# wexiangis/wmix

Hardware: AMD Instinct MI355X
Metric: 10 ms frames/s (higher is better)
Workload: dtype f32

## Files before the change

include/wmix_amd.h:

```cpp
#ifndef WMIX_AMD_H
#define WMIX_AMD_H

#include <stddef.h>
#include <stdint.h>

#ifdef __cplusplus
extern "C" {
#endif

#define WMX_EINVAL (-10001)
#define WMX_ENODEV (-10002)
#define WMX_ESTATE (-10003)
#define WMX_EHIP_BASE (-11000)
#define WMX_IS_HIP_ERROR(rc) ((rc) <= WMX_EHIP_BASE && (rc) > WMX_EHIP_BASE - 10000)

const char *wmx_last_error(void);
int wmx_device_count(void);
int wmx_handle_device(const void *handle);
int wmx_version(void);
const char *wmx_build_info(void);



#define WMX_LAW_A 0
// ... 125 lines not shown
wmx_ns *wmx_chain_ns(wmx_chain *h);
wmx_aec *wmx_chain_aec(wmx_chain *h);
wmx_agc *wmx_chain_agc(wmx_chain *h);
wmx_vad *wmx_chain_vad(wmx_chain *h);

typedef struct wmx_aecm wmx_aecm;
int wmx_aecm_create(wmx_aecm **out, int n_streams, int chn, int freq, int interval_ms);
int wmx_aecm_destroy(wmx_aecm *h);
int wmx_aecm_packet_samples(const wmx_aecm *h);
int wmx_aecm_state_bytes(const wmx_aecm *h);
int wmx_aecm_run(wmx_aecm *h, int mode, const int16_t *d_far, long far_packet_stride, const int16_t *d_near,
                 int16_t *d_out, int n_packets, long stream_stride, long packet_stride, int delay_ms, void *stream);
int wmx_aecm_create_cohorts(wmx_aecm **out, int n_streams, int chn, int freq, int interval_ms, int n_cohorts);
int wmx_aecm_cohorts(const wmx_aecm *h);
int wmx_aecm_reset_cohort(wmx_aecm *h, int cohort, void *stream);
int wmx_aecm_add_cohort(wmx_aecm *h, int *cohort, void *stream);
int wmx_aecm_retire_cohort(wmx_aecm *h, int cohort);
int wmx_aecm_coalesce(wmx_aecm *h, int max_pairs, int32_t *merged_from, int32_t *merged_into, int cap, int *n_merged, void *stream);
int wmx_aecm_live_cohorts(const wmx_aecm *h);
int wmx_aec_cohort_key(const wmx_aec *h, int cohort, int32_t *key11);
int wmx_aecm_cohort_key(const wmx_aecm *h, int cohort, int32_t *key8);
int wmx_aecm_reset_streams(wmx_aecm *h, const int32_t *idx, int n, int cohort, void *stream);
int wmx_aecm_set_active(wmx_aecm *h, const uint8_t *host_mask, void *stream);
int wmx_aecm_stream_state_bytes(const wmx_aecm *h);
int wmx_aecm_export_stream(wmx_aecm *h, int stream_index, void *host_blob);
int wmx_aecm_import_stream(wmx_aecm *h, int stream_index, const void *host_blob, int cohort);
int wmx_aecm_cohort_state_bytes(const wmx_aecm *h);
int wmx_aecm_export_cohort(wmx_aecm *h, int cohort, void *host_blob);
int wmx_aecm_import_cohort(wmx_aecm *h, int cohort, const void *host_blob);
int wmx_aecm_run_cohorts(wmx_aecm *h, int mode, const int16_t *d_far, long far_packet_stride, long far_group_stride,
                         const int16_t *d_near, int16_t *d_out, int n_packets, long stream_stride, long packet_stride,
                         const int32_t *delay_ms, const uint8_t *cohort_on, int32_t *cohort_rc, void *stream);
wmx_nsx *wmx_chain_nsx(wmx_chain *h);
wmx_aecm *wmx_chain_aecm(wmx_chain *h);

int wmx_pcm_zoom(int inChn, int inFreq, const int16_t *d_in, uint32_t inLen, int outChn, int outFreq, int16_t *d_out,
                 uint32_t out_capacity, long in_stride, long out_stride, int n_streams, uint32_t *out_len, void *stream);
typedef struct wmx_mix wmx_mix;
int wmx_mix_create(wmx_mix **out, int n_groups, int ring_chn, int ring_freq);
int wmx_mix_destroy(wmx_mix *m);
int wmx_mix_set(wmx_mix *m, uint32_t head_off, uint32_t tick, int reduce_mode);
int wmx_mix_set_play_correct(wmx_mix *m, uint32_t bytes);
int wmx_mix_ring_bytes(const wmx_mix *m);
int wmx_mix_load(wmx_mix *m, const int16_t *d_src, uint32_t srcU8Len, int freq, int channels, int sample, int n_src,
                 long group_stride, long source_stride, int reduce, uint32_t *head, uint32_t *tick, void *stream);
#define WMX_MIX_MAX_PARTIES 32
int wmx_mix_load_minus(wmx_mix *m, int parties, const int16_t *d_src, uint32_t srcU8Len, int freq, int channels, int sample,
                       long conf_stride, long source_stride, const uint8_t *d_mute, int reduce, uint32_t *head, uint32_t *tick,
                       void *stream);
int wmx_mix_set_conferences(wmx_mix *m, int n_conf, const int32_t *host_off, const int32_t *host_members, void *stream);
int wmx_mix_conferences(const wmx_mix *m);
int wmx_mix_load_minus_conf(wmx_mix *m, const int16_t *d_src, uint32_t srcU8Len, int freq, int channels, int sample,
                            long source_stride, const uint8_t *d_mute, int reduce, uint32_t *head, uint32_t *tick, void *stream);
int wmx_mix_select_speakers(wmx_mix *m, int parties, const int16_t *d_src, uint32_t srcU8Len, long conf_stride, long source_stride,
                            const uint8_t *d_mute, int max_speakers, uint32_t floor, int decay_shift, uint8_t *d_mute_out, void *stream);
int wmx_mix_select_speakers_conf(wmx_mix *m, const int16_t *d_src, uint32_t srcU8Len, long source_stride, const uint8_t *d_mute,
                                 int max_speakers, uint32_t floor, int decay_shift, uint8_t *d_mute_out, void *stream);
int wmx_mix_reset_speakers(wmx_mix *m, const int32_t *host_idx, int n, void *stream);
int wmx_mix_export_speakers(const wmx_mix *m, uint32_t *host_env, uint8_t *host_speaking, void *stream);
int wmx_mix_drain(wmx_mix *m, int16_t *d_out, uint32_t bytes, long out_stride, void *stream);
int wmx_mix_export(const wmx_mix *m, int group, int16_t *host_ring, uint32_t *head_off, uint32_t *tick);

#define WMX_MFFT_FFT 0
#define WMX_MFFT_FFTR 1
#define WMX_MFFT_IFFT 2
#define WMX_MFFT_IFFTR 3
int wmx_mfft(int kind, int n_batch, unsigned N, const float *d_in_re, const float *d_in_im, float *d_out_re,
             float *d_out_im, float *d_out_af, float *d_out_pf, void *stream);
int wmx_mfft_stream(int n_streams, const float *d_in, unsigned in_len, float *d_pool, unsigned st_len, float *d_out_af,
                    float *d_out_pf, void *stream);

typedef struct wmx_rtp wmx_rtp;
int wmx_rtp_create(wmx_rtp **out, int n_streams, int law);
int wmx_rtp_destroy(wmx_rtp *h);
int wmx_rtp_egress(wmx_rtp *h, int in_chn, int in_freq, const int16_t *d_pcm, uint32_t in_bytes, long pcm_stride, int out_chn,
                   int out_freq, uint8_t *d_packets, long packet_stride, uint32_t *packet_bytes, void *stream);
int wmx_rtp_ingest(int n_streams, const uint8_t *d_packets, long packet_stride, int16_t *d_pcm, long pcm_stride,
                   uint32_t *d_pcm_bytes, uint16_t *d_seq_raw, void *stream);
int wmx_rtp_export(wmx_rtp *h, int stream_index, uint16_t *seq, uint32_t *timestamp);

typedef struct wmx_pipe wmx_pipe;
int wmx_pipe_create(wmx_pipe **out, int n_streams, int slots, int law, int agc_value, unsigned stages);
int wmx_pipe_create_pcm(wmx_pipe **out, int n_streams, int slots, int chn, int freq, int interval_ms, int agc_value, unsigned stages);
int wmx_pipe_create_pcm_calls(wmx_pipe **out, int n_streams, int slots, int chn, int freq, int interval_ms, int agc_value, unsigned stages);
int wmx_pipe_destroy(wmx_pipe *h);
int wmx_pipe_slots(const wmx_pipe *h);
int wmx_pipe_datagram_bytes(const wmx_pipe *h);
uint8_t *wmx_pipe_in(wmx_pipe *h, int slot);
const uint8_t *wmx_pipe_out(wmx_pipe *h, int slot);
int16_t *wmx_pipe_far(wmx_pipe *h, int slot);
int wmx_pipe_submit(wmx_pipe *h, const int16_t *d_far, int *slot, void *stream);
int wmx_pipe_wait(wmx_pipe *h, int slot);
long wmx_pipe_failed_steps(const wmx_pipe *h);
int wmx_pipe_poll(wmx_pipe *h, int slot);
int wmx_pipe_step_resident(wmx_pipe *h, const uint8_t *d_in, long in_stride, const int16_t *d_far, uint8_t *d_out, long out_stride,
                           void *stream);
wmx_chain *wmx_pipe_chain(wmx_pipe *h);
wmx_rtp *wmx_pipe_senders(wmx_pipe *h);

typedef struct wmx_rt wmx_rt;
int wmx_rt_create_pcm(wmx_rt **out, long n_streams, int sub_batch, int slots, int chn, int freq, int interval_ms, int agc_value, unsigned stages);
int wmx_rt_create_rtp(wmx_rt **out, long n_streams, int sub_batch, int slots, int law, int agc_value, unsigned stages);
int wmx_rt_create_pcm_calls(wmx_rt **out, long n_streams, int sub_batch, int slots, int chn, int freq, int interval_ms, int agc_value, unsigned stages);
int wmx_rt_destroy(wmx_rt *h);
int wmx_rt_set_compute_streams(wmx_rt *h, int n);
int wmx_rt_batches(const wmx_rt *h);
int wmx_rt_batch_streams(const wmx_rt *h, int batch);
wmx_pipe *wmx_rt_pipe(wmx_rt *h, int batch);
int16_t *wmx_rt_far(wmx_rt *h, int slot);
int wmx_rt_submit(wmx_rt *h, const int16_t *d_far, int *slot, void *stream);
#define WMX_DROPPED 1
int wmx_rt_try_submit(wmx_rt *h, const int16_t *d_far, int *slot, void *stream);
long wmx_rt_dropped_ticks(const wmx_rt *h);
int wmx_rt_next_slot(const wmx_rt *h);
int wmx_rt_wait(wmx_rt *h);
int wmx_rt_poll(wmx_rt *h);
int wmx_rt_tick(wmx_rt *h, const int16_t *d_far, int *slot, void *stream);
int wmx_rt_step_resident(wmx_rt *h, uint8_t *d_rows, long stride, const int16_t *d_far, uint8_t *d_out, long out_stride, void *stream);

typedef struct wmx_pkgfifo wmx_pkgfifo;
int wmx_pkgfifo_create(wmx_pkgfifo **out, int n_streams, int n_slots, int pkg_bytes, int interval_ms, int frame_bytes);
int wmx_pkgfifo_destroy(wmx_pkgfifo *h);
int wmx_pkgfifo_add(wmx_pkgfifo *h, const uint8_t *d_pkgs, long stride, void *stream);
int wmx_pkgfifo_get(wmx_pkgfifo *h, uint8_t *d_out, long stride, int delayms, void *stream);

typedef struct wmx_tick wmx_tick;
int wmx_tick_create(wmx_tick **out, int n_groups, int rec_per_group, int chn, int freq, int interval_ms, int aec_delay_ms, int agc_value,
                    unsigned stages);
int wmx_tick_destroy(wmx_tick *h);
int wmx_tick_set_stages(wmx_tick *h, unsigned stages, int agc_value);
int wmx_tick_play_ns(wmx_tick *h, int on);
int wmx_tick_rw_test(wmx_tick *h, int on);
int wmx_tick_bridge(wmx_tick *h, int parties);
int wmx_tick_bridge_mute(wmx_tick *h, const uint8_t *host_mask, void *stream);
int wmx_tick_bridge_conferences(wmx_tick *h, int n_conf, const int32_t *host_off, const int32_t *host_members, void *stream);
int wmx_tick_bridge_speakers(wmx_tick *h, int max_speakers, uint32_t floor, int decay_shift);
int wmx_tick_bridge_speaking(wmx_tick *h, uint8_t *host_speaking, uint32_t *host_env, void *stream);
int wmx_tick_set_play_correct(wmx_tick *h, uint32_t bytes);
int wmx_tick_package_samples(const wmx_tick *h);
int wmx_tick_load(wmx_tick *h, const int16_t *d_src, uint32_t srcU8Len, int freq, int channels, int sample, int n_src, long group_stride,
                  long source_stride, int reduce, uint32_t *head, uint32_t *tick, void *stream);
int wmx_tick_play(wmx_tick *h, int16_t *d_play, long play_stride, void *stream);
const int16_t *wmx_tick_far(const wmx_tick *h);
int wmx_tick_record(wmx_tick *h, int16_t *d_rec, long rec_stride, int16_t *d_rec_1x8000, long out_stride, uint32_t out_capacity,
                    uint32_t *out_len, void *stream);
int wmx_tick_run(wmx_tick *h, int16_t *d_play, long play_stride, int16_t *d_rec, long rec_stride, int16_t *d_rec_1x8000, long out_stride,
                 uint32_t out_capacity, uint32_t *out_len, void *stream);
wmx_mix *wmx_tick_mix(wmx_tick *h);
wmx_chain *wmx_tick_chain(wmx_tick *h);
wmx_pkgfifo *wmx_tick_fifo(wmx_tick *h);

int wmx_debug_fft(int kind, int n_batch, void *d_data, int32_t *d_aux, void *stream);
int wmx_debug_ns_libm(int kind, const float *x, float *y, size_t n);
int wmx_debug_div(const float *d_a, const float *d_b, float *d_q_ordinary, float *d_q_ieee, size_t n, void *stream);
int wmx_debug_div_host(const float *a, const float *b, float *q, size_t n);
int wmx_debug_pow(const float *x, const float *e, float *y, size_t n);
int wmx_debug_pow_device(const float *d_x, const float *d_e, float *d_y, size_t n, void *stream);

#ifdef __cplusplus
}
#endif
#endif
```

tools_dev/ns_prof.py:

```python
import sys, ctypes; sys.path.insert(0,'.')
import numpy as np, torch
from wmix_amd import synth, _lib
from wmix_amd.ns import NsBatch
dev=torch.device('cuda:0'); S=int(sys.argv[1]) if len(sys.argv)>1 else 65536
import os
if os.environ.get('WMX_TOOL_LIB'): _lib.LIB_PATH=os.environ['WMX_TOOL_LIB']
lib=_lib.lib(); f=lib.wmx_debug_ns_prof; f.argtypes=[ctypes.c_void_p,ctypes.c_int]
nb=NsBatch(S,1,16000); nf=int(sys.argv[2]) if len(sys.argv)>2 else 260
x=synth.ns_input(7,64,nf,160)
d=torch.from_numpy(np.ascontiguousarray(x.reshape(64,nf,160).transpose(1,0,2))).to(dev).repeat(1,S//64,1).contiguous()
buf=(ctypes.c_ulonglong*16)()
for k in range(nf):
    if k==nf-8: f(buf,1)
    nb.process_packet_major(d[k:k+1])
f(buf,0); v=np.array(buf[:14],dtype=np.float64)
names=['load+window+energy1','fft fwd','spectrum+log','7 sums','noise est (quantiles)','startup/snr loop','3 sums+flat','lrt loop (log)','ksum+prior+exp loop','noise update+wiener','ifft','td+energy2','synth+hb','output']
for n,x in zip(names,v): print('%-24s %8.1f Mcyc %5.1f%%'%(n,x/1e6,100*x/v.sum()))
```

wmix_amd/csrc/ns.hip:

```cpp
#include <cmath>
#include <vector>
#include "stage_life.h"
#include "fft_ooura.h"
#include "libm_dev.h"
#include "ns_layout.h"

namespace wmx {
namespace {

constexpr int kStartupShort = 50;
constexpr int kStartupLong = 200;
constexpr int kHistBins = 1000;
constexpr int kUpdateWindow = 500;
constexpr int kStartBand = 5;

constexpr int kNsWavesPerBlock = 4;

template <int L>
struct NsConstLds {
    FftTables tab;
    float window[L];
    float logi[NsLayout<L>::MP];
    NsLibmTables lm;
};
template <int L>
struct alignas(16) NsWaveLds {
    static constexpr int MP = NsLayout<L>::MP;
    float fa[L];
    float magn[MP], lmagn[MP], noise[MP], snrp[MP], sprob[MP], pause[MP];
    float r0[MP], r1[MP], r2[MP];
#ifdef WMX_NS_PROF
    unsigned long long prof[16];
#endif
};
#ifdef WMX_NS_PROF
__device__ unsigned long long g_ns_prof[16];
#define NS_PROF(i)                                                         \
    do {                                                                   \
        const long long t_now = clock64();                                 \
        if (lane == 0) W.prof[i] += (unsigned long long)(t_now - prof_t0); \
        prof_t0 = clock64();                                               \
    } while (0)
#else
#define NS_PROF(i)
#endif
static_assert(2 * NsLayout<256>::MP >= 256 && 2 * NsLayout<128>::MP >= 128, "r0..r1 must hold L floats");

__device__ __forceinline__ float sat16f(float v) { return v > 32767.f ? 32767.f : (v < -32768.f ? -32768.f : v); }

__device__ __forceinline__ float sum_range(const float *x, int lo, int hi, int lane) {
    float acc = 0.f;
    int i = lo;
#pragma unroll 1
    for (; i < hi && (i & 3); i++) acc += x[i];
#pragma unroll 4
    for (; i + 8 <= hi; i += 8) {
        const float4 a = *reinterpret_cast<const float4 *>(x + i), b = *reinterpret_cast<const float4 *>(x + i + 4);
        acc += a.x;
        acc += a.y;
        acc += a.z;
        acc += a.w;
        acc += b.x;
        acc += b.y;
        acc += b.z;
        acc += b.w;
    }
#pragma unroll 1
    for (; i < hi; i++) acc += x[i];
    return acc;
}

template <int MP4>
__device__ __forceinline__ float sum_lanes(const float *mine) {
    float acc = 0.f;
#pragma unroll 4
    for (int i = 0; i < MP4; i += 2) {
        const float4 a = *reinterpret_cast<const float4 *>(mine + 4 * i);
        acc += a.x;
        acc += a.y;
        acc += a.z;
        acc += a.w;
        if (i + 1 < MP4) {
            const float4 b = *reinterpret_cast<const float4 *>(mine + 4 * i + 4);
            acc += b.x;
            acc += b.y;
            acc += b.z;
            acc += b.w;
        }
    }
    return acc;
}
__device__ __noinline__ static float tanh_call(float x, const NsLibmTables *m) { return fast_tanh(x, *m); }
__device__ __forceinline__ float lane_value(float v, int k) { return __int_as_float(__builtin_amdgcn_readlane(__float_as_int(v), k)); }

template <int L, int CHN>
__device__ void ns_frame(const NsConstLds<L> &K, NsWaveLds<L> &W, float *__restrict__ st, unsigned short *__restrict__ hist,
                         const int16_t *in, int16_t *out, const int pkg, const int lane_in) {
    using Y = NsLayout<L>;
    constexpr int chn = CHN;
    int lane = lane_in;
#define NS_RELANE() asm volatile("" : "+v"(lane))
    NS_RELANE();
#ifdef WMX_NS_PROF
    long long prof_t0 = clock64();
#endif
    constexpr int M = Y::M, B = Y::B, NT = L / 64, NC = L / 2;
    struct StF {
        GlobalF g;
        unsigned i;
        __device__ __forceinline__ operator float() const { return row_ld(g, i); }
        __device__ __forceinline__ void operator=(float v) const { row_st(g, i, v); }
    };
    struct StI {
        GlobalF g;
        unsigned i;
        __device__ __forceinline__ operator int() const { return __float_as_int(row_ld(g, i)); }
        __device__ __forceinline__ void operator=(int v) const { row_st(g, i, __int_as_float(v)); }
    };
    const GlobalF st_row = global_row(st, 0);
#define ST(idx) (StF{st_row, (unsigned)(idx)})
#define STI(idx) (StI{st_row, (unsigned)(idx)})
    float *tdst = W.r0;

    const float scv = lane < 24 ? ST(Y::SCALARS + lane) : 0.f;
#define SCF(f) lane_value(scv, Y::f - Y::SCALARS)
#define SCI(f) __float_as_int(lane_value(scv, Y::f - Y::SCALARS))
    float buf[NT], hb[NT], synt[NT];
#pragma unroll
    for (int k = 0; k < NT; k++) {
        const int i = lane + 64 * k;
        constexpr int KEEP = L - B;
        const bool all_old = 64 * k + 63 < KEEP, all_new = 64 * k >= KEEP;
        const bool is_old = all_old || (!all_new && i < KEEP);
        float o = 0.f, oh = 0.f;
        int16_t n = 0, nh = 0;
        if (!all_new) o = ST(Y::IN_BUF + (is_old ? i + B : 0));
        if (!all_old) n = in[(is_old ? 0 : i - KEEP) * chn];
        buf[k] = is_old ? o : (float)n;
        synt[k] = (64 * k < KEEP && i < KEEP) ? ST(Y::SYNT_BUF + (i < KEEP ? i : 0)) : 0.f;
        hb[k] = 0.f;
        if (chn == 2) {
            if (!all_new) oh = ST(Y::HB_BUF + (is_old ? i + B : 0));
            if (!all_old) nh = in[(is_old ? 0 : i - KEEP) * chn + 1];
            hb[k] = is_old ? oh : (float)nh;
        }
    }
#if defined(WMX_NS_EXP) && WMX_NS_EXP == 1
    constexpr int NI = M / 64;
#else
    constexpr int NI = (M + 63) / 64;
#endif
    float pf_quant[NI], pf_dens[NI][3], pf_lq[NI][3], pf_pause[NI];
#pragma unroll
    for (int k = 0; k < NI; k++) {
        const int b = lane + 64 * k < M ? lane + 64 * k : M - 1;
        pf_pause[k] = ST(Y::MAGN_AVG_PAUSE + b);
        pf_quant[k] = ST(Y::QUANTILE + b);
#pragma unroll
        for (int q = 0; q < 3; q++) {
            pf_dens[k][q] = ST(Y::DENSITY + q * Y::MP + b);
            pf_lq[k][q] = ST(Y::LQUANTILE + q * Y::MP + b);
        }
    }
    wave_sync();
#pragma unroll
    for (int k = 0; k < NT; k++) {
        const int i = lane + 64 * k;
        if (64 * k + 63 < B) continue;
        if (i >= B) {
            ST(Y::IN_BUF + i) = buf[k];
            if (chn == 2) ST(Y::HB_BUF + i) = hb[k];
        }
    }
#pragma unroll
    for (int k = 0; k < NT; k++) {
        const int i = lane + 64 * k;
        const float w = K.window[i] * buf[k];
        W.fa[i] = w;
        tdst[i] = w * w;
    }
    wave_sync();
    const float energy1 = sum_range(tdst, 0, L, lane);
    wave_sync();
    NS_PROF(0);

    float hb_gain = 1.f;
    const bool zero_frame = (energy1 == 0.0f);
    float t_re[(Y::M + 63) / 64], t_im[(Y::M + 63) / 64], t_prev[(Y::M + 63) / 64], t_snrq[(Y::M + 63) / 64];

    if (!zero_frame) {
        const int block_ind = SCI(S_BLOCK_IND) + 1;
        STI(Y::S_BLOCK_IND) = block_ind;
        const int update_flag = SCI(S_UPDATE_FLAG);
        const bool startup = block_ind < kStartupShort;
        const float overdrive = 1.1f, denoise_bound = 0.125f;

        NS_RELANE();
        rdft_forward<NC>(W.fa, &K.tab, lane);
        if (lane < Y::MP - M) W.r0[M + lane] = 0.f;
        NS_PROF(1);

        NS_RELANE();
#pragma unroll
        for (int k = 0; k < NI; k++) {
            const int b0 = lane + 64 * k;
            const bool ok = (64 * k + 63 < M) || b0 < M;
            const int b = ok ? b0 : M - 1;
            float re, im, mg;
            if (k == NI - 1) {
                re = W.fa[1];
                im = 0.f;
                mg = fabsf(re) + 1.f;
            } else {
                const float a0 = W.fa[2 * b], a1 = W.fa[2 * b + 1];
                const bool dc = k == 0 && b == 0;
                re = a0;
                im = dc ? 0.f : a1;
                const float g = sqrtf(re * re + im * im) + 1.f;
                mg = dc ? fabsf(re) + 1.f : g;
            }
            const float lm = fast_log_ge1(mg, K.lm);
            const float pz = pf_pause[k];
            t_re[k] = re;
            t_im[k] = im;
            if (!ok) continue;
            W.magn[b] = mg;
            W.lmagn[b] = lm;
            W.pause[b] = pz;
            W.r0[b] = re * re + im * im;
            W.r1[b] = b >= kStartBand ? K.logi[b] * lm : 0.f;
            W.r2[b] = b >= 1 ? lm : 0.f;
            W.snrp[b] = b >= kStartBand ? lm : 0.f;
        }
        wave_sync();
        NS_PROF(2);
        float signal_energy, sum_magn, flat_num, avg_pause, sum_log_magn = 0.f, sum_log_i_log_magn = 0.f;
        {
            const float *mine =
                lane == 1 ? W.magn : (lane == 2 ? W.r2 : (lane == 3 ? W.pause : (lane == 4 ? W.snrp : (lane == 5 ? W.r1 : W.r0))));
            const float acc = sum_lanes<Y::MP / 4>(mine);
            signal_energy = lane_value(acc, 0);
            sum_magn = lane_value(acc, 1);
            flat_num = lane_value(acc, 2);
            avg_pause = lane_value(acc, 3);
            if (startup) {
                sum_log_magn = lane_value(acc, 4);
                sum_log_i_log_magn = lane_value(acc, 5);
            }
        }
        const float magn0 = W.magn[0];
        wave_sync();
        NS_PROF(3);
        signal_energy = signal_energy / ((float)M);

        NS_RELANE();
        int updates = SCI(S_UPDATES);
        if (updates < kStartupLong) updates++;
        STI(Y::S_UPDATES) = updates;
        const int cnt0 = SCI(S_COUNTER + 0), cnt1 = SCI(S_COUNTER + 1), cnt2 = SCI(S_COUNTER + 2);
        float pf_nprev[NI], pf_mprev[NI], pf_smooth[NI], pf_lrt[NI];
#pragma unroll
        for (int k = 0; k < NI; k++) {
            const int b = lane + 64 * k < M ? lane + 64 * k : M - 1;
            pf_nprev[k] = ST(Y::NOISE_PREV + b);
            pf_mprev[k] = ST(Y::MAGN_PREV + b);
            pf_smooth[k] = ST(Y::SMOOTH + b);
            pf_lrt[k] = ST(Y::LOG_LRT + b);
        }
#pragma unroll
        for (int k = 0; k < NI; k++) {
            const int b0 = lane + 64 * k;
            const bool ok = (64 * k + 63 < M) || b0 < M;
            const int b = ok ? b0 : M - 1;
            const float lm = W.lmagn[b];
            float quant = pf_quant[k], lq = 0.f;
#pragma unroll
            for (int q = 0; q < 3; q++) {
                const int cnt = q == 0 ? cnt0 : (q == 1 ? cnt1 : cnt2);
                const float c1 = (float)(cnt + 1), cf = (float)cnt;
                float dens = pf_dens[k][q];
                lq = pf_lq[k][q];
                float delta;
                if (dens > 1.0f)
                    delta = div_ordinary(40.f * 1.f, dens);
                else
                    delta = 40.f;
                lq += div_ordinary(lm > lq ? 0.25f * delta : -((1.f - 0.25f) * delta), c1);
                if (fabsf(lm - lq) < 0.01f) {
                    dens = div_ordinary(cf * dens + 1.f / (2.f * 0.01f), c1);
                    if (ok) ST(Y::DENSITY + q * Y::MP + b) = dens;
                }
                if (ok) ST(Y::LQUANTILE + q * Y::MP + b) = lq;
                if (cnt >= kStartupLong && updates >= kStartupLong) quant = fast_exp(lq, K.lm);
            }
            if (updates < kStartupLong) quant = fast_exp(lq, K.lm);
            if (ok) {
                if (updates < kStartupLong || cnt0 >= kStartupLong || cnt1 >= kStartupLong || cnt2 >= kStartupLong) ST(Y::QUANTILE + b) = quant;
                W.noise[b] = quant;
            }
        }
        STI(Y::S_COUNTER + 0) = cnt0 >= kStartupLong ? 1 : cnt0 + 1;
        STI(Y::S_COUNTER + 1) = cnt1 >= kStartupLong ? 1 : cnt1 + 1;
        STI(Y::S_COUNTER + 2) = cnt2 >= kStartupLong ? 1 : cnt2 + 1;

        NS_RELANE();
        NS_PROF(4);
        if (startup) {
            const float white = SCF(S_WHITE) + sum_magn / ((float)M) * overdrive;
            ST(Y::S_WHITE) = white;
            const float sum_log_i = K.logi[Y::MP - 2], sum_log_i_sq = K.logi[Y::MP - 1];
            float t1 = sum_log_i_sq * ((float)(M - kStartBand));
            t1 -= (sum_log_i * sum_log_i);
            float t2 = (sum_log_i_sq * sum_log_magn - sum_log_i * sum_log_i_log_magn);
            float t3 = t2 / t1;
            if (t3 < 0.f) t3 = 0.f;
            const float pink_num = SCF(S_PINK_NUM) + t3;
            ST(Y::S_PINK_NUM) = pink_num;
            t2 = (sum_log_i * sum_log_magn);
            t2 -= ((float)(M - kStartBand)) * sum_log_i_log_magn;
            t3 = t2 / t1;
            if (t3 < 0.f) t3 = 0.f;
            if (t3 > 1.f) t3 = 1.f;
            const float pink_exp = SCF(S_PINK_EXP) + t3;
            ST(Y::S_PINK_EXP) = pink_exp;
            float pnum = 0.0f, pexp = 0.0f;
            if (pink_exp > 0.f) {
                pnum = exp_d(pink_num / (float)(block_ind + 1));
                pnum *= (float)(block_ind + 1);
                pexp = pink_exp / (float)(block_ind + 1);
            }
#pragma unroll 1
            for (int b = lane; b < M; b += 64) {
                float pn;
                if (pink_exp == 0.f) {
                    pn = white;
                } else {
                    const float band = (float)(b < kStartBand ? kStartBand : b);
                    pn = div_pow_d(pnum, band, pexp);
                }
                W.r1[b] = pn;
                float nz = W.noise[b];
                nz *= (float)(block_ind);
                const float t = pn * (float)(kStartupShort - block_ind);
                nz += (t / (float)(block_ind + 1));
                nz /= (float)kStartupShort;
                W.noise[b] = nz;
            }
        }
        float feat_norm = SCF(S_FEAT_NORM);
        if (block_ind < kStartupLong) {
            feat_norm *= (float)block_ind;
            feat_norm += signal_energy;
            feat_norm /= (float)(block_ind + 1);
        }

        NS_RELANE();
        avg_pause = avg_pause / ((float)M);
        const float avg_magn = sum_magn / ((float)M);
#pragma unroll
        for (int k = 0; k < NI; k++) {
            const int b0 = lane + 64 * k;
            const bool ok = (64 * k + 63 < M) || b0 < M;
            const int b = ok ? b0 : M - 1;
            const float mg = W.magn[b], nz = W.noise[b];
            const float np = pf_nprev[k];
            const float pe = div_ordinary(pf_mprev[k], np + 0.0001f) * pf_smooth[k];
            float sq = 0.f;
            if (mg > nz) sq = div_ordinary(mg, nz + 0.0001f) - 1.f;
            const float dm = mg - avg_magn, dp = W.pause[b] - avg_pause;
            t_prev[k] = pe;
            t_snrq[k] = sq;
            if (!ok) continue;
            W.snrp[b] = 0.98f * pe + (1.f - 0.98f) * sq;
            W.r0[b] = dm * dp;
            W.r2[b] = dp * dp;
            W.lmagn[b] = dm * dm;
        }
        wave_sync();
        NS_PROF(5);
        float feat_flat = SCF(S_FEAT_FLAT);
        {
            float den = sum_magn;
            den -= magn0;
            den = den / (float)M;
            const float num = flat_num / (float)M;
            const float tmp = fast_exp(num, K.lm) / den;
            feat_flat += 0.3f * (tmp - feat_flat);
        }
        float cov, var_pause, var_magn;
        {
            const float acc = sum_lanes<Y::MP / 4>(lane == 1 ? W.r2 : (lane == 2 ? W.lmagn : W.r0));
            cov = lane_value(acc, 0);
            var_pause = lane_value(acc, 1);
            var_magn = lane_value(acc, 2);
        }
        wave_sync();
        NS_PROF(6);
        cov = cov / ((float)M);
        var_pause = var_pause / ((float)M);
        var_magn = var_magn / ((float)M);
        float feat_acc = SCF(S_FEAT_ACC) + signal_energy;
        float feat_diff = SCF(S_FEAT_DIFF);
        {
            float d = var_magn - (cov * cov) / (var_pause + 0.0001f);
            d = d / (feat_norm + 0.0001f);
            feat_diff += 0.3f * (d - feat_diff);
        }
        float feat_lrt = SCF(S_FEAT_LRT);
        float thr_lrt = SCF(S_THR_LRT), thr_flat = SCF(S_THR_FLAT), thr_diff = SCF(S_THR_DIFF);
        float w_lrt = SCF(S_W_LRT), w_flat = SCF(S_W_FLAT), w_diff = SCF(S_W_DIFF);
        if (update_flag >= 1) {
            const int countdown = SCI(S_COUNTDOWN) - 1;
            if (countdown > 0) {
                if (lane == 0) {
                    auto bump = [&](int i) { atomicAdd(reinterpret_cast<unsigned *>(hist) + (i >> 1), (i & 1) ? 0x10000u : 1u); };
                    if ((feat_lrt < kHistBins * 0.1f) && (feat_lrt >= 0.0f)) bump((int)(feat_lrt / 0.1f));
                    if ((feat_flat < kHistBins * 0.05f) && (feat_flat >= 0.0f)) bump(kHistBins + (int)(feat_flat / 0.05f));
                    if ((feat_diff < kHistBins * 0.1f) && (feat_diff >= 0.0f)) bump(2 * kHistBins + (int)(feat_diff / 0.1f));
                }
                STI(Y::S_COUNTDOWN) = countdown;
            } else {
                unsigned hc_[3][8];
#pragma unroll
                for (int w_ = 0; w_ < 3; w_++) {
                    const unsigned *hsrc_ = reinterpret_cast<const unsigned *>(hist + w_ * kHistBins);
#pragma unroll
                    for (int q = 0; q < 8; q++) {
                        const int d_ = 64 * q + lane;
                        const unsigned v_ = hsrc_[d_ < kHistBins / 2 ? d_ : 0];
                        hc_[w_][q] = d_ < kHistBins / 2 ? v_ : 0u;
                    }
                }
#define NS_WALK(which, ...)                                                                                        \
    {                                                                                                              \
        constexpr int CH_ = 2 * L, QPC_ = L / 64, NCH_ = 8 / QPC_;  \
        const unsigned(&c_)[8] = hc_[which];                                                                       \
        _Pragma("unroll") for (int part_ = 0; part_ < NCH_; part_++) {                                             \
            unsigned *stage_ = reinterpret_cast<unsigned *>(W.fa);                                                 \
            _Pragma("unroll") for (int q = 0; q < QPC_; q++) stage_[64 * q + lane] = c_[QPC_ * part_ + q];         \
            wave_sync();                                                                                           \
            const unsigned short *h16_ = reinterpret_cast<const unsigned short *>(W.fa);                           \
            _Pragma("unroll 1") for (int base = CH_ * part_; base < CH_ * part_ + CH_ && base < kHistBins; base += 64) { \
                const int hv = (int)h16_[base - CH_ * part_ + lane];                                               \
                unsigned long long m = __builtin_amdgcn_ballot_w64(hv != 0);                                       \
                while (m) {                                                                                        \
                    const int j = __builtin_ctzll(m);                                                              \
                    m &= m - 1;                                                                                    \
                    const int i = base + j, h = __builtin_amdgcn_readlane(hv, j);                                  \
                    __VA_ARGS__                                                                                    \
                }                                                                                                  \
            }                                                                                                      \
            wave_sync();                                                                                           \
        }                                                                                                          \
    }
                static_assert(L == 128 || L == 256, "the staging above is sized for these");
                float avg = 0.0f, avg_compl = 0.0f, avg_sq = 0.0f;
                int num = 0;
                NS_WALK(0, {
                    const float mid = ((float)i + 0.5f) * 0.1f;
                    if (mid <= 1.f) {
                        avg += h * mid;
                        num += h;
                    }
                    avg_sq += h * mid * mid;
                    avg_compl += h * mid;
                })
                if (num > 0) avg = avg / ((float)num);
                avg_compl = avg_compl / ((float)kUpdateWindow);
                avg_sq = avg_sq / ((float)kUpdateWindow);
                const float fluct = avg_sq - avg * avg_compl;
                if (fluct < 0.05f) {
                    thr_lrt = 1.f;
                } else {
                    thr_lrt = 1.2f * avg;
                    if (thr_lrt < 0.2f) thr_lrt = 0.2f;
                    if (thr_lrt > 1.f) thr_lrt = 1.f;
                }
                int w1a = 0, w2a = 0, w1b = 0, w2b = 0;
                float p1a = 0.0f, p2a = 0.0f, p1b = 0.0f, p2b = 0.0f;
                {
                    int max1 = 0, max2 = 0;
                    NS_WALK(1, {
                        const float mid = ((float)i + 0.5f) * 0.05f;
                        if (h > max1) {
                            max2 = max1, w2a = w1a, p2a = p1a;
                            max1 = h, w1a = h, p1a = mid;
                        } else if (h > max2) {
                            max2 = h, w2a = h, p2a = mid;
                        }
                    })
                }
                {
                    int max1 = 0, max2 = 0;
                    NS_WALK(2, {
                        const float mid = ((float)i + 0.5f) * 0.1f;
                        if (h > max1) {
                            max2 = max1, w2b = w1b, p2b = p1b;
                            max1 = h, w1b = h, p1b = mid;
                        } else if (h > max2) {
                            max2 = h, w2b = h, p2b = mid;
                        }
                    })
                }
#undef NS_WALK
                const int thres_weight = 150;
                int use_flat = 1, use_diff = 1;
                if ((fabsf(p2a - p1a) < 2 * 0.05f) && (w2a > 0.5f * w1a)) {
                    w1a += w2a;
                    p1a = 0.5f * (p1a + p2a);
                }
                if (w1a < thres_weight || p1a < 0.6f) use_flat = 0;
                if (use_flat == 1) {
                    thr_flat = 0.9f * p1a;
                    if (thr_flat < 0.1f) thr_flat = 0.1f;
                    if (thr_flat > 0.95f) thr_flat = 0.95f;
                }
                if ((fabsf(p2b - p1b) < 2 * 0.1f) && (w2b > 0.5f * w1b)) {
                    w1b += w2b;
                    p1b = 0.5f * (p1b + p2b);
                }
                thr_diff = 1.2f * p1b;
                if (w1b < thres_weight) use_diff = 0;
                if (thr_diff < 0.16f) thr_diff = 0.16f;
                if (thr_diff > 1.f) thr_diff = 1.f;
                if (fluct < 0.05f) use_diff = 0;
                const float fsum = (float)(1 + use_flat + use_diff);
                w_lrt = 1.f / fsum;
                w_flat = ((float)use_flat) / fsum;
                w_diff = ((float)use_diff) / fsum;
                wave_sync();
                for (int i = lane; i < 3 * kHistBins; i += 64) hist[i] = 0;
                STI(Y::S_COUNTDOWN) = kUpdateWindow;
                if (update_flag == 1) {
                    STI(Y::S_UPDATE_FLAG) = 0;
                } else {
                    feat_acc = feat_acc / ((float)kUpdateWindow);
                    feat_norm = 0.5f * (feat_acc + feat_norm);
                    feat_acc = 0.f;
                }
                ST(Y::S_THR_LRT) = thr_lrt;
                ST(Y::S_THR_FLAT) = thr_flat;
                ST(Y::S_THR_DIFF) = thr_diff;
                ST(Y::S_W_LRT) = w_lrt;
                ST(Y::S_W_FLAT) = w_flat;
                ST(Y::S_W_DIFF) = w_diff;
            }
        }
        ST(Y::S_FEAT_FLAT) = feat_flat;
        ST(Y::S_FEAT_DIFF) = feat_diff;
        ST(Y::S_FEAT_NORM) = feat_norm;
        ST(Y::S_FEAT_ACC) = feat_acc;

        NS_RELANE();
#pragma unroll
        for (int k = 0; k < NI; k++) {
            const int b0 = lane + 64 * k;
            const bool ok = (64 * k + 63 < M) || b0 < M;
            const int b = ok ? b0 : M - 1;
            const float sp = W.snrp[b];
            const float t1 = 1.f + 2.f * sp;
            const float t2 = div_ordinary(2.f * sp, t1 + 0.0001f);
            const float bessel = (t_snrq[k] + 1.f) * t2;
            float v = pf_lrt[k];
            v += 0.5f * (bessel - fast_log_ge1(t1, K.lm) - v);
            if (!ok) continue;
            ST(Y::LOG_LRT + b) = v;
            W.r0[b] = v;
        }
        wave_sync();
        NS_PROF(7);
        float ksum = sum_range(W.r0, 0, M, lane);
        ksum = ksum / (float)(M);
        feat_lrt = ksum;
        ST(Y::S_FEAT_LRT) = feat_lrt;
        float prior = SCF(S_PRIOR);
        {
            float width = 4.0f;
            if (ksum < thr_lrt) width = 2.f * 4.0f;
            const float a0 = width * (ksum - thr_lrt);
            width = 4.0f;
            if (feat_flat > thr_flat) width = 2.f * 4.0f;
            const float a1 = (float)1 * width * (thr_flat - feat_flat);
            width = 4.0f;
            if (feat_diff < thr_diff) width = 2.f * 4.0f;
            const float a2 = width * (feat_diff - thr_diff);
            const float th = fast_tanh(lane == 1 ? a1 : (lane == 2 ? a2 : a0), K.lm);
            const float ind0 = 0.5f * (lane_value(th, 0) + 1.f);
            const float ind1 = 0.5f * (lane_value(th, 1) + 1.f);
            const float ind2 = 0.5f * (lane_value(th, 2) + 1.f);
            const float ind = w_lrt * ind0 + w_flat * ind1 + w_diff * ind2;
            prior += 0.1f * (ind - prior);
            if (prior > 1.f) prior = 1.f;
            if (prior < 0.01f) prior = 0.01f;
            ST(Y::S_PRIOR) = prior;
        }
        const float gain_prior = (1.f - prior) / (prior + 0.0001f);
#pragma unroll
        for (int k = 0; k < NI; k++) {
            const int b0 = lane + 64 * k;
            const bool ok = (64 * k + 63 < M) || b0 < M;
            const int b = ok ? b0 : M - 1;
            float inv = fast_exp(-W.r0[b], K.lm);
            inv = gain_prior * inv;
            const float spb = 1.f / (1.f + inv);
            if (ok) W.sprob[b] = spb;
        }
        wave_sync();
        NS_PROF(8);
        NS_RELANE();
#pragma unroll
        for (int k = 0; k < NI; k++) {
            const int b0 = lane + 64 * k;
            const bool ok = (64 * k + 63 < M) || b0 < M;
            const int b = ok ? b0 : M - 1;
            const float ps = W.sprob[b], pn = 1.f - ps, mg = W.magn[b], np = pf_nprev[k];
            float gamma_old = 0.9f;
            if (b > 0 && W.sprob[b - 1] > 0.2f) gamma_old = 0.99f;
            const float tmp = gamma_old * np + (1.f - gamma_old) * (pn * mg + ps * np);
            float gamma = 0.9f;
            if (ps > 0.2f) gamma = 0.99f;
            if (ps < 0.2f) {
                float pz = W.pause[b];
                pz += 0.05f * (mg - pz);
                if (ok) ST(Y::MAGN_AVG_PAUSE + b) = pz;
            }
            float nz;
            if (gamma == gamma_old) {
                nz = tmp;
            } else {
                nz = gamma * np + (1.f - gamma) * (pn * mg + ps * np);
                if (tmp < nz) nz = tmp;
            }
            float init_est = 0.f;
            if (startup) {
                init_est = ST(Y::INIT_MAGN + b) + mg;
                if (ok) ST(Y::INIT_MAGN + b) = init_est;
            }
            float cur = 0.f;
            if (mg > nz) cur = div_ordinary(mg, nz + 0.0001f) - 1.f;
            const float snr = 0.98f * t_prev[k] + (1.f - 0.98f) * cur;
            float f = div_ordinary(snr, overdrive + snr);
            if (f < denoise_bound) f = denoise_bound;
            if (f > 1.f) f = 1.f;
            if (startup) {
                float ft = (init_est - overdrive * W.r1[b]);
                ft /= (init_est + 0.0001f);
                if (ft < denoise_bound) ft = denoise_bound;
                if (ft > 1.f) ft = 1.f;
                f *= (float)(block_ind);
                ft *= (float)(kStartupShort - block_ind);
                f += ft;
                f /= (float)(kStartupShort);
            }
            const float re = t_re[k] * f, im = t_im[k] * f;
            if (!ok) continue;
            ST(Y::SMOOTH + b) = f;
            ST(Y::MAGN_PREV + b) = mg;
            ST(Y::NOISE_PREV + b) = nz;
            W.snrp[b] = f;
            if (b == 0)
                W.fa[0] = re;
            else if (b == M - 1)
                W.fa[1] = re;
            else {
                W.fa[2 * b] = re;
                W.fa[2 * b + 1] = im;
            }
        }
        wave_sync();
        NS_PROF(9);
        NS_RELANE();
        rdft_inverse<NC>(W.fa, &K.tab, lane);
        NS_PROF(10);
        float td[NT];
#pragma unroll
        for (int k = 0; k < NT; k++) {
            const int i = lane + 64 * k;
            td[k] = W.fa[i] * (2.f / L);
            tdst[i] = td[k] * td[k];
        }
        wave_sync();
        NS_PROF(11);
        float factor = 1.f;
        if (block_ind > kStartupLong) {
            const float energy2 = sum_range(tdst, 0, L, lane);
            float gain = sqrtf(energy2 / (energy1 + 1.f));
            float factor1 = 1.f, factor2 = 1.f;
            if (gain > 0.5f) {
                factor1 = 1.f + 1.3f * (gain - 0.5f);
                if (gain * factor1 > 1.f) factor1 = 1.f / gain;
            }
            if (gain < 0.5f) {
                if (gain <= denoise_bound) gain = denoise_bound;
                factor2 = 1.f - 0.3f * (0.5f - gain);
            }
            factor = prior * factor1 + (1.f - prior) * factor2;
        }
#pragma unroll
        for (int k = 0; k < NT; k++) {
            const int i = lane + 64 * k;
            const float w = K.window[i] * td[k];
            synt[k] += factor * w;
        }
        if (chn == 2) {
            constexpr int D = M / 4;
            float avg_prob = sum_range(W.sprob, M - D - 1, M - 1, lane);
            avg_prob = avg_prob / ((float)D);
            avg_prob *= sum_magn / sum_magn;
            float avg_gain = sum_range(W.snrp, M - D - 1, M - 1, lane);
            avg_gain = avg_gain / ((float)D);
            const float t = 2.f * avg_prob - 1.f;
            const float gain_mod = 0.5f * (1.f + tanh_call(1.0f * t, &K.lm));
            float g = 0.5f * gain_mod + 0.5f * avg_gain;
            if (avg_prob >= 0.5f) g = 0.25f * gain_mod + 0.75f * avg_gain;
            g = g * 1.0f;
            if (g < denoise_bound) g = denoise_bound;
            if (g > 1.f) g = 1.f;
            hb_gain = g;
        }
        wave_sync();
        NS_PROF(12);
    }

        NS_RELANE();
#pragma unroll
    for (int k = 0; k < NT; k++) {
        const int i = lane + 64 * k;
        if (i >= B) ST(Y::SYNT_BUF + i - B) = synt[k];
        tdst[i] = sat16f(synt[k]);
        if (chn == 2) W.fa[i] = zero_frame ? sat16f(hb[k]) : sat16f(hb_gain * hb[k]);
    }
    wave_sync();
    for (int i = lane; i < pkg; i += 64) {
        const float lo = (i < B) ? tdst[i] : 0.f;
        out[i * chn] = (int16_t)lo;
        if (chn == 2) out[i * chn + 1] = (int16_t)((i < B) ? W.fa[i] : 0.f);
    }
    wave_sync();
    NS_PROF(13);
#undef NS_RELANE
#undef SCF
#undef SCI
#undef ST
#undef STI
}

#ifndef WMX_NS_W128
#define WMX_NS_W128 7
#endif
#ifndef WMX_NS_W256
#define WMX_NS_W256 5
#endif
template <int L>
struct NsOcc {
    static constexpr int kWaves = L == 128 ? WMX_NS_W128 : WMX_NS_W256;
};
template <int L, int CHN>
__global__ __launch_bounds__(64 * kNsWavesPerBlock) __attribute__((amdgpu_waves_per_eu(NsOcc<L>::kWaves, NsOcc<L>::kWaves))) void ns_kernel(float *__restrict__ state, unsigned short *__restrict__ hists,
                                                                      const float *__restrict__ consts, const int16_t *in, int16_t *out,
                                                                      int n_streams, int n_packets, long stream_stride,
                                                                      long packet_stride, int pkg, const uint8_t *__restrict__ active) {
    using Y = NsLayout<L>;
    __shared__ NsConstLds<L> K;
    __shared__ NsWaveLds<L> Wv[kNsWavesPerBlock];
    {
        float *dst = reinterpret_cast<float *>(&K);
        constexpr int NCONST = sizeof(NsConstLds<L>) / 4, NIT = (NCONST + 64 * kNsWavesPerBlock - 1) / (64 * kNsWavesPerBlock);
        float c[NIT];
#pragma unroll
        for (int k = 0; k < NIT; k++) {
            const int i = threadIdx.x + 64 * kNsWavesPerBlock * k;
            c[k] = consts[i < NCONST ? i : 0];
        }
#pragma unroll
        for (int k = 0; k < NIT; k++) {
            const int i = threadIdx.x + 64 * kNsWavesPerBlock * k;
            if (i < NCONST) dst[i] = c[k];
        }
    }
    __syncthreads();
    const int lane = threadIdx.x & 63;
    const int wave = __builtin_amdgcn_readfirstlane(threadIdx.x >> 6);
    const int sidx = blockIdx.x * kNsWavesPerBlock + wave;
    if (!stream_active(active, sidx, n_streams)) return;
    float *st = state + (size_t)sidx * Y::WORDS;
    unsigned short *hist = hists + (size_t)sidx * 3 * kHistBins;
    {
        float *wb = Wv[wave].magn;
        constexpr int NARR = 9;
        if (lane < NARR * (Y::MP - Y::M)) wb[(lane / (Y::MP - Y::M)) * Y::MP + Y::M + lane % (Y::MP - Y::M)] = 0.f;
    }
#ifdef WMX_NS_PROF
    if (lane < 16) Wv[wave].prof[lane] = 0;
#endif
    for (int p = 0; p < n_packets; p++) {
        const size_t off = (size_t)sidx * stream_stride + (size_t)p * packet_stride;
        ns_frame<L, CHN>(K, Wv[wave], st, hist, in + off, out + off, pkg, lane);
    }
#ifdef WMX_NS_PROF
    if (lane < 16) atomicAdd(&g_ns_prof[lane], Wv[wave].prof[lane]);
#endif
}
#ifdef WMX_NS_PROF
extern "C" int wmx_debug_ns_prof(unsigned long long *out16, int reset) {
    (void)hipDeviceSynchronize();
    (void)hipMemcpyFromSymbol(out16, HIP_SYMBOL(g_ns_prof), sizeof(unsigned long long) * 16);
    if (reset) {
        unsigned long long z[16] = {0};
        (void)hipMemcpyToSymbol(HIP_SYMBOL(g_ns_prof), z, sizeof(z));
    }
    return 0;
}
#endif

}
}

struct wmx_ns {
    int device;
    int n_streams, chn, freq, L, pkg;
    float *d_state;
    unsigned short *d_hist;
    float *d_consts;
    float *d_tmpl;
    size_t words;
    wmx::StreamLife life;
};

namespace {

template <int L>
void build_ns_template(std::vector<float> &st, std::vector<float> &consts) {
    using Y = wmx::NsLayout<L>;
    st.assign(Y::WORDS, 0.f);
    int *sti = reinterpret_cast<int *>(st.data());
    for (int q = 0; q < 3; q++)
        for (int b = 0; b < Y::M; b++) {
            st[Y::LQUANTILE + q * Y::MP + b] = 8.f;
// ... 61 lines not shown
        wmx::set_error("wmx_ns_create: unsupported n_streams=%d chn=%d freq=%d", n_streams, chn, freq);
        return WMX_EINVAL;
    }
    wmx_ns *h = new wmx_ns();
    if ((h->device = wmx::current_device()) < 0) {
        delete h;
        return WMX_ENODEV;
    }
    h->n_streams = n_streams;
    h->chn = chn;
    h->freq = freq;
    h->L = (freq == 8000) ? 128 : 256;
    h->pkg = freq / 1000 * 10;
    std::vector<float> st, consts;
    if (h->L == 128)
        build_ns_template<128>(st, consts);
    else
        build_ns_template<256>(st, consts);
    h->words = st.size();
    WMX_CREATE_TRY(wmx_ns_destroy(h), hipMalloc(&h->d_state, h->words * sizeof(float) * (size_t)n_streams));
    WMX_CREATE_TRY(wmx_ns_destroy(h), hipMalloc(&h->d_hist, (size_t)n_streams * 3 * 1000 * sizeof(unsigned short)));
    WMX_CREATE_TRY(wmx_ns_destroy(h), hipMalloc(&h->d_consts, consts.size() * sizeof(float)));
    WMX_CREATE_TRY(wmx_ns_destroy(h), hipMalloc(&h->d_tmpl, st.size() * sizeof(float)));
    WMX_CREATE_TRY(wmx_ns_destroy(h), hipMemcpy(h->d_consts, consts.data(), consts.size() * sizeof(float), hipMemcpyHostToDevice));
    WMX_CREATE_TRY(wmx_ns_destroy(h), hipMemcpy(h->d_tmpl, st.data(), st.size() * sizeof(float), hipMemcpyHostToDevice));
    WMX_CREATE_TRY(wmx_ns_destroy(h), hipMemset(h->d_hist, 0, (size_t)n_streams * 3 * 1000 * sizeof(unsigned short)));
    hipLaunchKernelGGL(ns_fill_state, dim3(1024), dim3(256), 0, nullptr, h->d_state, h->d_tmpl, (int)h->words, n_streams);
    WMX_CREATE_TRY(wmx_ns_destroy(h), hipGetLastError());
    WMX_CREATE_TRY(wmx_ns_destroy(h), hipDeviceSynchronize());
    *out = h;
    return 0;
}

int wmx_ns_destroy(wmx_ns *h) {
    WMX_ON_DEVICE(h);
    if (!h) return 0;
    if (h->d_state) (void)hipFree(h->d_state);
    if (h->d_hist) (void)hipFree(h->d_hist);
    if (h->d_consts) (void)hipFree(h->d_consts);
    if (h->d_tmpl) (void)hipFree(h->d_tmpl);
    h->life.release();
    delete h;
    return 0;
}

int wmx_ns_reset_streams(wmx_ns *h, const int32_t *idx, int n, void *stream) {
    return wmx::reset_streams(h, idx, n, stream, [=](hipStream_t s, const int32_t *d_idx) {
        const unsigned grid = (unsigned)(n < 4096 ? n : 4096);
        hipLaunchKernelGGL((wmx::fill_rows_idx<float>), dim3(grid), dim3(256), 0, s, h->d_state, (const float *)h->d_tmpl, (int)h->words, d_idx, n);
        hipLaunchKernelGGL((wmx::fill_rows_idx<unsigned short>), dim3(grid), dim3(256), 0, s, h->d_hist, (const unsigned short *)nullptr, 3000, d_idx, n);
        WMX_LAUNCH_CHECK();
        return 0;
    });
}

int wmx_ns_set_active(wmx_ns *h, const uint8_t *host_mask, void *stream) { return wmx::set_active(h, host_mask, stream); }

static wmx::StreamBlob ns_blob(const wmx_ns *h) {
    return {wmx::blob_tag("NS  "), wmx::blob_layout((uint32_t)h->L, 1), {{h->d_state, 4, h->words}, {h->d_hist, 2, 3000}}, 0};
}
int wmx_ns_stream_state_bytes(const wmx_ns *h) { return wmx::stream_state_bytes(h, ns_blob); }
int wmx_ns_export_stream(wmx_ns *h, int stream_index, void *host_blob) { return wmx::export_stream(h, stream_index, host_blob, ns_blob); }
int wmx_ns_import_stream(wmx_ns *h, int stream_index, const void *host_blob) { return wmx::import_stream(h, stream_index, host_blob, ns_blob); }

int wmx_ns_packet_samples(const wmx_ns *h) { return h ? h->pkg * h->chn : WMX_EINVAL; }
int wmx_ns_state_words(const wmx_ns *h) { return h ? (int)h->words : WMX_EINVAL; }

int wmx_ns_export_state(const wmx_ns *h, int stream_index, float *host_words, unsigned short *host_hist) {
    WMX_ON_DEVICE(h);
    if (!h || stream_index < 0 || stream_index >= h->n_streams) return WMX_EINVAL;
    WMX_HIP(hipDeviceSynchronize());
    if (host_words)
        WMX_HIP(hipMemcpy(host_words, h->d_state + (size_t)stream_index * h->words, h->words * sizeof(float), hipMemcpyDeviceToHost));
    if (host_hist)
        WMX_HIP(hipMemcpy(host_hist, h->d_hist + (size_t)stream_index * 3000, 3000 * sizeof(unsigned short), hipMemcpyDeviceToHost));
    return 0;
}

int wmx_ns_process(wmx_ns *h, const int16_t *d_in, int16_t *d_out, int n_packets, long stream_stride,
                   long packet_stride, void *stream) {
    WMX_ON_DEVICE(h);
    if (!h || n_packets < 0) {
        wmx::set_error("wmx_ns_process: bad argument");
        return WMX_EINVAL;
    }
    if (n_packets == 0) return 0;
    if (!d_in || !d_out) {
        wmx::set_error("wmx_ns_process: null buffer");
        return WMX_EINVAL;
    }
    const int per_pkt = h->pkg * h->chn;
    if (packet_stride < per_pkt || (h->n_streams > 1 && stream_stride < per_pkt)) {
        wmx::set_error("wmx_ns_process: strides (%ld, %ld) smaller than a packet (%d samples)", stream_stride, packet_stride, per_pkt);
        return WMX_EINVAL;
    }
    const unsigned grid = (unsigned)((h->n_streams + wmx::kNsWavesPerBlock - 1) / wmx::kNsWavesPerBlock);
    hipStream_t s = wmx::as_stream(stream);
#define NS_LAUNCH(LL, CC)                                                                                                  \
    hipLaunchKernelGGL((wmx::ns_kernel<LL, CC>), dim3(grid), dim3(64 * wmx::kNsWavesPerBlock), 0, s, h->d_state, h->d_hist, \
                       h->d_consts, d_in, d_out, h->n_streams, n_packets, stream_stride, packet_stride, h->pkg, h->life.d_active)
    if (h->L == 128) {
        if (h->chn == 1)
            NS_LAUNCH(128, 1);
        else
            NS_LAUNCH(128, 2);
    } else {
        if (h->chn == 1)
            NS_LAUNCH(256, 1);
        else
            NS_LAUNCH(256, 2);
    }
#undef NS_LAUNCH
    WMX_LAUNCH_CHECK();
    return 0;
}

}

namespace wmx {
namespace {
__global__ void div_debug_kernel(const float *a, const float *b, float *q_ordinary, float *q_ieee, size_t n) {
    for (size_t i = blockIdx.x * (size_t)blockDim.x + threadIdx.x; i < n; i += (size_t)gridDim.x * blockDim.x) {
        q_ordinary[i] = div_ordinary(a[i], b[i]);
        q_ieee[i] = a[i] / b[i];
    }
}
}
}
extern "C" int wmx_debug_div(const float *d_a, const float *d_b, float *d_q_ordinary, float *d_q_ieee, size_t n, void *stream) {
    if (!d_a || !d_b || !d_q_ordinary || !d_q_ieee) return WMX_EINVAL;
    if (n == 0) return 0;
    hipLaunchKernelGGL(wmx::div_debug_kernel, dim3(4096), dim3(256), 0, wmx::as_stream(stream), d_a, d_b, d_q_ordinary, d_q_ieee, n);
    WMX_LAUNCH_CHECK();
    return 0;
}
extern "C" int wmx_debug_div_host(const float *a, const float *b, float *q, size_t n) {
    if (!a || !b || !q) return WMX_EINVAL;
    for (size_t i = 0; i < n; i++) q[i] = wmx::div_ordinary(a[i], b[i]);
    return 0;
}

extern "C" int wmx_debug_ns_libm(int kind, const float *x, float *y, size_t n) {
    static wmx::NsLibmTables tab;
    static bool init = false;
    if (!init) {
        wmx::ns_libm_tables(&tab);
        init = true;
    }
    if (!x || !y || kind < 0 || kind > 2) return WMX_EINVAL;
    for (size_t i = 0; i < n; i++)
        y[i] = kind == 0 ? wmx::fast_log_ge1(x[i], tab) : (kind == 1 ? wmx::fast_exp(x[i], tab) : wmx::fast_tanh(x[i], tab));
    return 0;
}
```

Before: 60.03 million.

## Batch noise-suppression reductions and replace energy sum with ballot zero gate

Replaces the full energy1 reduction with a wave ballot that only tests whether any windowed sample is nonzero. The actual energy1 sum is deferred to the late path, where it is combined with energy2 in a single multi-lane reduction. The LRT loop moves earlier and its ksum is folded into the existing covariance/variance multi-lane sum, removing a separate reduction and its barrier. Divisions by M are applied lane-wise after the sums. A debug export for the window table is also added.

```diff
diff --git a/include/wmix_amd.h b/include/wmix_amd.h
--- a/include/wmix_amd.h
+++ b/include/wmix_amd.h
@@ -301,6 +301,7 @@
 
 int wmx_debug_fft(int kind, int n_batch, void *d_data, int32_t *d_aux, void *stream);
 int wmx_debug_ns_libm(int kind, const float *x, float *y, size_t n);
+int wmx_debug_ns_window(int L, float *host_window);
 int wmx_debug_div(const float *d_a, const float *d_b, float *d_q_ordinary, float *d_q_ieee, size_t n, void *stream);
 int wmx_debug_div_host(const float *a, const float *b, float *q, size_t n);
 int wmx_debug_pow(const float *x, const float *e, float *y, size_t n);
diff --git a/tools_dev/ns_prof.py b/tools_dev/ns_prof.py
--- a/tools_dev/ns_prof.py
+++ b/tools_dev/ns_prof.py
@@ -14,5 +14,5 @@
     if k==nf-8: f(buf,1)
     nb.process_packet_major(d[k:k+1])
 f(buf,0); v=np.array(buf[:14],dtype=np.float64)
-names=['load+window+energy1','fft fwd','spectrum+log','7 sums','noise est (quantiles)','startup/snr loop','3 sums+flat','lrt loop (log)','ksum+prior+exp loop','noise update+wiener','ifft','td+energy2','synth+hb','output']
+names=['load+window+zero gate','fft fwd','spectrum+log','6 sums','noise est (quantiles)','startup/snr loop+lrt loop (log)','4 sums+flat','features+histograms','prior+exp loop','noise update+wiener','ifft','td','2 energies+synth+hb','output']
 for n,x in zip(names,v): print('%-24s %8.1f Mcyc %5.1f%%'%(n,x/1e6,100*x/v.sum()))
diff --git a/wmix_amd/csrc/ns.hip b/wmix_amd/csrc/ns.hip
--- a/wmix_amd/csrc/ns.hip
+++ b/wmix_amd/csrc/ns.hip
@@ -172,20 +172,21 @@
             if (chn == 2) ST(Y::HB_BUF + i) = hb[k];
         }
     }
+    float e1[NT];
+    bool any_term = false;
 #pragma unroll
     for (int k = 0; k < NT; k++) {
         const int i = lane + 64 * k;
         const float w = K.window[i] * buf[k];
         W.fa[i] = w;
-        tdst[i] = w * w;
-    }
-    wave_sync();
-    const float energy1 = sum_range(tdst, 0, L, lane);
+        e1[k] = w * w;
+        any_term |= e1[k] != 0.0f;
+    }
     wave_sync();
     NS_PROF(0);
 
     float hb_gain = 1.f;
-    const bool zero_frame = (energy1 == 0.0f);
+    const bool zero_frame = __builtin_amdgcn_ballot_w64(any_term) == 0;
     float t_re[(Y::M + 63) / 64], t_im[(Y::M + 63) / 64], t_prev[(Y::M + 63) / 64], t_snrq[(Y::M + 63) / 64];
 
     if (!zero_frame) {
@@ -234,15 +235,17 @@
         }
         wave_sync();
         NS_PROF(2);
-        float signal_energy, sum_magn, flat_num, avg_pause, sum_log_magn = 0.f, sum_log_i_log_magn = 0.f;
+        float signal_energy, sum_magn, avg_magn, flat_mean, avg_pause, sum_log_magn = 0.f, sum_log_i_log_magn = 0.f;
         {
             const float *mine =
                 lane == 1 ? W.magn : (lane == 2 ? W.r2 : (lane == 3 ? W.pause : (lane == 4 ? W.snrp : (lane == 5 ? W.r1 : W.r0))));
             const float acc = sum_lanes<Y::MP / 4>(mine);
-            signal_energy = lane_value(acc, 0);
+            const float mean = acc / ((float)M);
+            signal_energy = lane_value(mean, 0);
             sum_magn = lane_value(acc, 1);
-            flat_num = lane_value(acc, 2);
-            avg_pause = lane_value(acc, 3);
+            avg_magn = lane_value(mean, 1);
+            flat_mean = lane_value(mean, 2);
+            avg_pause = lane_value(mean, 3);
             if (startup) {
                 sum_log_magn = lane_value(acc, 4);
                 sum_log_i_log_magn = lane_value(acc, 5);
@@ -251,7 +254,6 @@
         const float magn0 = W.magn[0];
         wave_sync();
         NS_PROF(3);
-        signal_energy = signal_energy / ((float)M);
 
         NS_RELANE();
         int updates = SCI(S_UPDATES);
@@ -306,7 +308,7 @@
         NS_RELANE();
         NS_PROF(4);
         if (startup) {
-            const float white = SCF(S_WHITE) + sum_magn / ((float)M) * overdrive;
+            const float white = SCF(S_WHITE) + avg_magn * overdrive;
             ST(Y::S_WHITE) = white;
             const float sum_log_i = K.logi[Y::MP - 2], sum_log_i_sq = K.logi[Y::MP - 1];
             float t1 = sum_log_i_sq * ((float)(M - kStartBand));
@@ -355,8 +357,6 @@
         }
 
         NS_RELANE();
-        avg_pause = avg_pause / ((float)M);
-        const float avg_magn = sum_magn / ((float)M);
 #pragma unroll
         for (int k = 0; k < NI; k++) {
             const int b0 = lane + 64 * k;
@@ -371,10 +371,24 @@
             t_prev[k] = pe;
             t_snrq[k] = sq;
             if (!ok) continue;
-            W.snrp[b] = 0.98f * pe + (1.f - 0.98f) * sq;
             W.r0[b] = dm * dp;
             W.r2[b] = dp * dp;
             W.lmagn[b] = dm * dm;
+        }
+#pragma unroll
+        for (int k = 0; k < NI; k++) {
+            const int b0 = lane + 64 * k;
+            const bool ok = (64 * k + 63 < M) || b0 < M;
+            const int b = ok ? b0 : M - 1;
+            const float sp = 0.98f * t_prev[k] + (1.f - 0.98f) * t_snrq[k];
+            const float t1 = 1.f + 2.f * sp;
+            const float t2 = div_ordinary(2.f * sp, t1 + 0.0001f);
+            const float bessel = (t_snrq[k] + 1.f) * t2;
+            float v = pf_lrt[k];
+            v += 0.5f * (bessel - fast_log_ge1(t1, K.lm) - v);
+            if (!ok) continue;
+            ST(Y::LOG_LRT + b) = v;
+            W.sprob[b] = v;
         }
         wave_sync();
         NS_PROF(5);
@@ -383,22 +397,20 @@
             float den = sum_magn;
             den -= magn0;
             den = den / (float)M;
-            const float num = flat_num / (float)M;
-            const float tmp = fast_exp(num, K.lm) / den;
+            const float tmp = fast_exp(flat_mean, K.lm) / den;
             feat_flat += 0.3f * (tmp - feat_flat);
         }
-        float cov, var_pause, var_magn;
+        float cov, var_pause, var_magn, ksum;
         {
-            const float acc = sum_lanes<Y::MP / 4>(lane == 1 ? W.r2 : (lane == 2 ? W.lmagn : W.r0));
-            cov = lane_value(acc, 0);
-            var_pause = lane_value(acc, 1);
-            var_magn = lane_value(acc, 2);
+            const float acc = sum_lanes<Y::MP / 4>(lane == 1 ? W.r2 : (lane == 2 ? W.lmagn : (lane == 3 ? W.sprob : W.r0)));
+            const float mean = acc / ((float)M);
+            cov = lane_value(mean, 0);
+            var_pause = lane_value(mean, 1);
+            var_magn = lane_value(mean, 2);
+            ksum = lane_value(mean, 3);
         }
         wave_sync();
         NS_PROF(6);
-        cov = cov / ((float)M);
-        var_pause = var_pause / ((float)M);
-        var_magn = var_magn / ((float)M);
         float feat_acc = SCF(S_FEAT_ACC) + signal_energy;
         float feat_diff = SCF(S_FEAT_DIFF);
         {
@@ -552,25 +564,7 @@
         ST(Y::S_FEAT_ACC) = feat_acc;
 
         NS_RELANE();
-#pragma unroll
-        for (int k = 0; k < NI; k++) {
-            const int b0 = lane + 64 * k;
-            const bool ok = (64 * k + 63 < M) || b0 < M;
-            const int b = ok ? b0 : M - 1;
-            const float sp = W.snrp[b];
-            const float t1 = 1.f + 2.f * sp;
-            const float t2 = div_ordinary(2.f * sp, t1 + 0.0001f);
-            const float bessel = (t_snrq[k] + 1.f) * t2;
-            float v = pf_lrt[k];
-            v += 0.5f * (bessel - fast_log_ge1(t1, K.lm) - v);
-            if (!ok) continue;
-            ST(Y::LOG_LRT + b) = v;
-            W.r0[b] = v;
-        }
-        wave_sync();
         NS_PROF(7);
-        float ksum = sum_range(W.r0, 0, M, lane);
-        ksum = ksum / (float)(M);
         feat_lrt = ksum;
         ST(Y::S_FEAT_LRT) = feat_lrt;
         float prior = SCF(S_PRIOR);
@@ -600,7 +594,7 @@
             const int b0 = lane + 64 * k;
             const bool ok = (64 * k + 63 < M) || b0 < M;
             const int b = ok ? b0 : M - 1;
-            float inv = fast_exp(-W.r0[b], K.lm);
+            float inv = fast_exp(-W.sprob[b], K.lm);
             inv = gain_prior * inv;
             const float spb = 1.f / (1.f + inv);
             if (ok) W.sprob[b] = spb;
@@ -683,7 +677,11 @@
         NS_PROF(11);
         float factor = 1.f;
         if (block_ind > kStartupLong) {
-            const float energy2 = sum_range(tdst, 0, L, lane);
+#pragma unroll
+            for (int k = 0; k < NT; k++) W.fa[lane + 64 * k] = e1[k];
+            wave_sync();
+            const float acc = sum_lanes<L / 4>(lane == 1 ? W.fa : tdst);
+            const float energy2 = lane_value(acc, 0), energy1 = lane_value(acc, 1);
             float gain = sqrtf(energy2 / (energy1 + 1.f));
             float factor1 = 1.f, factor2 = 1.f;
             if (gain > 0.5f) {
@@ -1051,3 +1049,14 @@
         y[i] = kind == 0 ? wmx::fast_log_ge1(x[i], tab) : (kind == 1 ? wmx::fast_exp(x[i], tab) : wmx::fast_tanh(x[i], tab));
     return 0;
 }
+
+extern "C" int wmx_debug_ns_window(int L, float *host_window) {
+    if (!host_window || (L != 128 && L != 256)) return WMX_EINVAL;
+    std::vector<float> st, consts;
+    if (L == 128)
+        build_ns_template<128>(st, consts);
+    else
+        build_ns_template<256>(st, consts);
+    std::memcpy(host_window, consts.data() + wmx::kFftTableWords, sizeof(float) * L);
+    return 0;
+}
```

Measured after the change: 61.80 million, median of 6. 2.9% higher.
